# anzeA/Tarok

Measured on AMD Instinct MI355X. Metric: env steps/sec at 65 536 parallel 4-player games; 1/2/4/8 MI355X, higher is better.
Workload: dtype u64

## Files before the change

tarok_amd/csrc/tarok_device.h:

```cpp
#pragma once
#include <hip/hip_runtime.h>
#include <stdint.h>

typedef unsigned long long u64;
typedef uint32_t u32;

#define TK_VGPR_BUDGET(B) __attribute__((amdgpu_num_vgpr((B) - 1)))
#define TK_KERNEL(threads, B) __global__ __launch_bounds__(threads) TK_VGPR_BUDGET(B)
#define TK_VGPR_STR2(x) #x
#define TK_VGPR_STR(x) TK_VGPR_STR2(x)
#define TK_VGPR_TOP(B, TOP)                                                                                           \
    do {                                                                                                              \
        static_assert((B) % 8 == 0 && (B) <= 256 && (TOP) == (B) - 1, "TK_VGPR_TOP(B, B - 1), B a multiple of 8");     \
        asm volatile("" ::: "v" TK_VGPR_STR(TOP));                                                                    \
    } while (0)

#define TK_BIT(i) (1ULL << (i))
#define TK_DECK ((1ULL << 54) - 1)
#define TK_TAROK (((1ULL << 22) - 1) << 32)
#define TK_PAGAT TK_BIT(32)
#define TK_V5 (TK_BIT(7) | TK_BIT(15) | TK_BIT(23) | TK_BIT(31) | TK_BIT(32) | TK_BIT(52) | TK_BIT(53))
#define TK_V4 (TK_BIT(6) | TK_BIT(14) | TK_BIT(22) | TK_BIT(30))
#define TK_V3 (TK_BIT(5) | TK_BIT(13) | TK_BIT(21) | TK_BIT(29))
#define TK_V2 (TK_BIT(4) | TK_BIT(12) | TK_BIT(20) | TK_BIT(28))
// ... 106 lines not shown
        u32 gs = group_size(g.contract);
        return talon_all(g) & ~ids_mask(g.talon, (int)(g.tl * gs), (int)gs);
    }
    return talon_all(g);
}

__device__ __forceinline__ int prestej(u64 m) {
    u32 lo = TK_LO(m), hi = TK_HI(m);
    u32 n = (u32)__popc(lo) + (u32)__popc(hi);
    u32 v = n + (u32)__popc(lo & 0xF0F0F0F0u) + (u32)__popc(lo & 0xE0E0E0E0u) + (u32)__popc(lo & 0xC0C0C0C0u) +
            (u32)__popc(lo & 0x80808080u) + 4u * (u32)__popc(hi & 0x300001u);
    u32 q = (n * 43u) >> 7;
    return (int)(v - 2 * q - (n != 3 * q ? 1u : 0u));
}

__device__ __forceinline__ u32 tk_zero_mask(u32 x) { return (u32)((int)__builtin_amdgcn_sad_u8(x, 0u, ~0u) >> 31); }
__device__ __forceinline__ u64 legal_mask(u64 hand, bool has_lead, u32 lead, u32 contract) {
    u32 hl = TK_LO(hand), hh = TK_HI(hand);
    u32 lm = has_lead ? ~0u : 0u;
    u32 tarok_led = (u32)((int)(lead << 26) >> 31);
    u32 s = TK_BITOP3(hl, 0xFFu << (lead & 24), tarok_led, a_ & b_ & ~c_) & lm;
    u32 zs = tk_zero_mask(s);
    u32 zt = tk_zero_mask(hh) | ~lm;
    u32 bl = s | TK_BITOP3(hl, zs, zt, a_ & b_ & c_);
    u32 bh = hh & zs;
    u32 kf = (0x281u >> contract) & 1u;
    u32 only_pagat = tk_zero_mask(bl | (bh & ~1u));
    return TK_U64(bl, TK_BITOP3(bh, kf, only_pagat, a_ & ~(b_ & ~c_)));
}

__device__ __forceinline__ u64 legal_mask_follow(u64 hand, u32 lead, u32 contract, u32 &hi_sel) {
    u32 hl = TK_LO(hand), hh = TK_HI(hand);
    u32 tarok_led = (u32)((int)(lead << 26) >> 31);
    u32 s = TK_BITOP3(hl, 0xFFu << (lead & 24), tarok_led, a_ & b_ & ~c_);
    u32 zs = tk_zero_mask(s);
    u32 zt = tk_zero_mask(hh);
    u32 bl = s | TK_BITOP3(hl, zs, zt, a_ & b_ & c_);
    u32 bh = hh & zs;
    u32 kf = (0x281u >> contract) & 1u;
    u32 only_pagat = tk_zero_mask(bl | (bh & ~1u));
    hi_sel = TK_BITOP3(zs, zt, zt, a_ & ~b_);           TK_KEEP_VGPR(hi_sel);
    return TK_U64(bl, TK_BITOP3(bh, kf, only_pagat, a_ & ~(b_ & ~c_)));
}

#define TK_FAM_LUT 0xA0000281u
#define TK_FAM_MASK 0x80400001u
struct FamilyWord { u32 w; };
struct LeadWord { u32 m; };
__device__ __forceinline__ FamilyWord family_word(u32 contract) {
    u32 w = (TK_FAM_LUT >> contract) & TK_FAM_MASK;     TK_KEEP_VGPR(w);
    return FamilyWord{w};
}
__device__ __forceinline__ LeadWord lead_word(u32 lead) {
    u32 tarok_led = (u32)((int)(lead << 26) >> 31);     TK_KEEP_VGPR(tarok_led);
    return LeadWord{(0xFFu << (lead & 24)) & ~tarok_led};
}
__device__ __forceinline__ u64 legal_mask(u64 hand, FamilyWord fam) {
    u32 hl = TK_LO(hand), hh = TK_HI(hand);
    u32 only_pagat = tk_zero_mask(hl | (hh & ~1u));
    return TK_U64(hl, TK_BITOP3(hh, fam.w, only_pagat, a_ & ~(b_ & ~c_)));
}
__device__ __forceinline__ u64 legal_mask_follow(u64 hand, LeadWord lead, FamilyWord fam, u32 &hi_sel) {
    u32 hl = TK_LO(hand), hh = TK_HI(hand);
    u32 s = hl & lead.m;
    u32 zs = tk_zero_mask(s);
    u32 zt = tk_zero_mask(hh);
    u32 bl = s | TK_BITOP3(hl, zs, zt, a_ & b_ & c_);
    u32 bh = hh & zs;
    u32 only_pagat = tk_zero_mask(bl | (bh & ~1u));
    hi_sel = TK_BITOP3(zs, zt, zt, a_ & ~b_);           TK_KEEP_VGPR(hi_sel);
    return TK_U64(bl, TK_BITOP3(bh, fam.w, only_pagat, a_ & ~(b_ & ~c_)));
}

__device__ __forceinline__ u64 legal_now(const Game &g) {
    u32 seat = (g.leader + g.nt) & 3;
    return legal_mask(hand_of(g, seat), g.nt != 0, g.trick & 63, g.contract);
}

template <bool IN_PLAY = false>
__device__ __forceinline__ u64 obs_word_with(const Game &g, bool finished_now, u64 legal) {
    u64 o = legal;
    o |= (u64)((g.leader + g.nt) & 3) << 54;
    o |= (u64)(g.trick_no * 4 + g.nt) << 56;
    if (IN_PLAY) o |= (u64)(finished_now ? 1u : 0u) << 62;
    else if (finished_now || g.phase == TK_PHASE_DONE) o |= 1ULL << 62;
    o |= (u64)g.error << 63;
    return o;
}

#define TK_OBS_CARD ((1u << 30) + 1u)
__device__ __forceinline__ u32 obs_carry(u32 seat, u32 pos) { return (seat << 30) | pos; }
__device__ __forceinline__ u32 obs_carry_hi(u32 carry) { return (carry >> 8) | (carry << 24); }
__device__ __forceinline__ u64 obs_word_with(u32 carry, u32 error, u32 fin01, u64 legal) {
    return legal | ((u64)(obs_carry_hi(carry) | (fin01 << 30) | (error << 31)) << 32);
}

__device__ __forceinline__ u32 obs_carry(u32 seat, u32 pos, u32 error) { return (error << 7) | obs_carry(seat, pos); }
__device__ __forceinline__ u32 obs_carry_ma(u32 carry) { return (u32)((int)(carry << 1) >> 31); }
__device__ __forceinline__ u32 obs_carry_mb(u32 carry) { return (u32)((int)carry >> 31); }
__device__ __forceinline__ u64 obs_word_with(u32 carry_with_error, u32 fin01, u64 legal) {
    return legal | ((u64)(obs_carry_hi(carry_with_error) | (fin01 << 30)) << 32);
}

__device__ __forceinline__ u64 obs_word(const Game &g, bool finished_now) {
    bool play = g.phase == TK_PHASE_PLAY;
    u64 o = play ? legal_now(g) : 0;
    o |= (u64)((g.leader + g.nt) & 3) << 54;
    o |= (u64)(g.trick_no * 4 + g.nt) << 56;
    if (finished_now || g.phase == TK_PHASE_DONE) o |= 1ULL << 62;
    o |= (u64)g.error << 63;
    return o;
}

__device__ __forceinline__ u64 pack_scores(int s0, int s1, int s2, int s3) {
    return (u64)(uint16_t)(int16_t)s0 | ((u64)(uint16_t)(int16_t)s1 << 16) |
           ((u64)(uint16_t)(int16_t)s2 << 32) | ((u64)(uint16_t)(int16_t)s3 << 48);
}

__device__ __forceinline__ u64 score_game(const Game &g) {
    bool klop = g.contract == TK_KLOP;
    u64 p0 = pile_of<0>(g), p1 = pile_of<1>(g), p2 = pile_of<2>(g), p3 = pile_of<3>(g);
    u32 t0 = (u32)((int)(g.team << 31) >> 31), t1 = (u32)((int)(g.team << 30) >> 31);
    u32 t2 = (u32)((int)(g.team << 29) >> 31), t3 = (u32)((int)(g.team << 28) >> 31);
    u32 xl = TK_BITOP3(TK_LO(g.A), t1, t0, (a_ & b_) | (~a_ & c_)), yl = TK_BITOP3(TK_LO(g.A), t3, t2, (a_ & b_) | (~a_ & c_));
    u32 xh = TK_BITOP3(TK_HI(g.A), t1, t0, (a_ & b_) | (~a_ & c_)), yh = TK_BITOP3(TK_HI(g.A), t3, t2, (a_ & b_) | (~a_ & c_));
    u32 tl = TK_BITOP3(TK_LO(g.B), yl, xl, (a_ & b_) | (~a_ & c_)) & TK_LO(g.C);
    u32 th = TK_BITOP3(TK_HI(g.B), yh, xh, (a_ & b_) | (~a_ & c_)) & TK_HI(g.C);
    u64 t = TK_U64(tl, th);
    u32 kb = g.king * 8 + 7, d = g.declarer;
    bool king_taken = ((TK_LO(g.C) >> kb) & 1) && ((TK_LO(g.A) >> kb) & 1) == (d & 1) && ((TK_LO(g.B) >> kb) & 1) == (d >> 1);
    bool alone_with_king = !klop && g.contract != TK_SOLO_BREZ && __popc(g.team) == 1 && has_king(g.contract) && king_taken;
    if (alone_with_king) t |= talon_unowned(g);
    int c0 = prestej(klop ? p0 : t), c1 = prestej(klop ? p1 : 0), c2 = prestej(klop ? p2 : 0), c3 = prestej(klop ? p3 : 0);
    bool over = c0 > 35 || c1 > 35 || c2 > 35 || c3 > 35;
    int d0 = c0 - 35, ad = d0 < 0 ? -d0 : d0;
    int r = 5 * (int)(((u32)(ad + 2) * 205u) >> 10);
    if (d0 < 0) r = -r;
    int c = 10 * (int)g.contract;
    int sc = (c0 > 35 ? c : -c) + r;
    int s0 = klop ? (over ? 0 : -c0) : ((g.team & 1) ? sc : 0);
    int s1 = klop ? (over ? 0 : -c1) : ((g.team & 2) ? sc : 0);
    int s2 = klop ? (over ? 0 : -c2) : ((g.team & 4) ? sc : 0);
    int s3 = klop ? (over ? 0 : -c3) : ((g.team & 8) ? sc : 0);
    return pack_scores(s0, s1, s2, s3);
}

__device__ __forceinline__ u64 berac_scores(const Game &g) {
    int v = g.contract == TK_BERAC ? 70 : 90;
    int sc = g.leader == g.declarer ? -v : v;
    u32 d = g.declarer;
    return pack_scores(d == 0 ? sc : 0, d == 1 ? sc : 0, d == 2 ? sc : 0, d == 3 ? sc : 0);
}

template <bool TRUSTED = false, bool DEFER = false, bool CARRIED = false>
__device__ __forceinline__ int apply_step(Game &g, u32 a, u64 &scores, u32 &trick_info, bool want_tv = true, const u64 *c_lead = nullptr,
                                          FamilyWord fam = FamilyWord{0u}, LeadWord lead = LeadWord{0u}) {
    if (!TRUSTED) {
        u64 legal = legal_now(g);
        bool ok = a < 54 && ((legal >> (a & 63)) & 1);
        g.error = ok ? g.error : 1u;
        if (!ok) return -1;
    }
    g.C |= 1ULL << a;
    g.trick |= a << (6 * g.nt);
    g.nt++;
    if (g.nt < 4) return 0;
    u64 tm;
    if (c_lead) tm = g.C ^ *c_lead;
    else {
        u32 c0 = g.trick & 63, c1 = (g.trick >> 6) & 63, c2 = (g.trick >> 12) & 63, c3 = (g.trick >> 18) & 63;
        tm = (1ULL << c0) | (1ULL << c1) | (1ULL << c2) | (1ULL << c3);
    }
    u32 th = TK_HI(tm), tl_ = TK_LO(tm) & (CARRIED ? lead.m : (0xFFu << (g.trick & 24)));
    u32 zt = tk_zero_mask(th);
    u32 wbit = 31u - (u32)__builtin_clz(TK_BITOP3(th, tl_, zt, (a_ & ~c_) | (b_ & c_)));
    u32 aw = TK_BITOP3(TK_HI(g.A), TK_LO(g.A), zt, (a_ & ~c_) | (b_ & c_)), bw = TK_BITOP3(TK_HI(g.B), TK_LO(g.B), zt, (a_ & ~c_) | (b_ & c_));
    u32 ws = __builtin_amdgcn_ubfe(aw, wbit, 1) | (__builtin_amdgcn_ubfe(bw, wbit, 1) << 1);
    {
        u32 gift = CARRIED ? min(g.tl, fam.w >> 31) : (tk_zero_mask(g.contract) & ((g.tl + 7u) >> 3));
        g.tl -= gift;
        u64 gb = 1ULL << ((u32)(g.talon >> (6 * g.tl)) & 63u);
        u32 gm = 0u - gift;
        tm |= TK_U64(TK_LO(gb) & gm, TK_HI(gb) & gm);
    }
    {
        u32 m1 = (u32)((int)(ws << 31) >> 31), m2 = (u32)((int)(ws << 30) >> 31);
        g.A = TK_U64(TK_BITOP3(TK_LO(g.A), TK_LO(tm), m1, (a_ & ~b_) | (b_ & c_)), TK_BITOP3(TK_HI(g.A), TK_HI(tm), m1, (a_ & ~b_) | (b_ & c_)));
        g.B = TK_U64(TK_BITOP3(TK_LO(g.B), TK_LO(tm), m2, (a_ & ~b_) | (b_ & c_)), TK_BITOP3(TK_HI(g.B), TK_HI(tm), m2, (a_ & ~b_) | (b_ & c_)));
    }
    if (want_tv) {
        u32 tv = (u32)(popc64(tm) + popc64(tm & (TK_V2 | TK_V3 | TK_V4 | TK_V5)) + popc64(tm & (TK_V3 | TK_V4 | TK_V5)) +
                       popc64(tm & (TK_V4 | TK_V5)) + popc64(tm & TK_V5)) - 2;
        trick_info = 0x8000u | (tv << 4) | ws;
    }
    g.leader = ws; g.nt = 0; g.trick = 0; g.trick_no++;
    u32 berac01 = CARRIED ? __builtin_amdgcn_ubfe(fam.w, 22u, 1u) : ((0x280u >> g.contract) & 1u);
    u32 over01 = ((g.trick_no + 4u) >> 4) | (berac01 & tk_zero_mask(ws ^ g.declarer));
    if (!DEFER) {
        if (over01) scores = berac01 ? berac_scores(g) : score_game(g);
    }
    g.phase |= over01;
    return (int)over01;
}

__device__ __forceinline__ u64 final_scores(const Game &g) {
    return (g.contract == TK_BERAC || g.contract == TK_ODPRTI_BERAC) ? berac_scores(g) : score_game(g);
}

__device__ __forceinline__ void setup_game(Game &g, u64 h0, u64 h1, u64 h2, u64 h3, u64 talon36,
                                           u32 contract, u32 declarer, u32 king) {
    g.A = h1 | h3; g.B = h2 | h3;
    g.talon = talon36;
    u64 tal = ids_mask(talon36, 0, 6);
    g.C = tal;
    g.trick = 0; g.nt = 0; g.trick_no = 0; g.error = 0;
    g.contract = contract; g.declarer = declarer;
    g.king = has_king(contract) ? king : 0;
    g.leader = (contract == TK_BERAC || contract == TK_ODPRTI_BERAC) ? declarer : 0;
    if (contract == TK_KLOP) {
        g.team = 0; g.tl = 6;
    } else {
        u32 team = 1u << declarer;
        if (has_king(contract)) {
            u64 kb = 1ULL << (king * 8 + 7);
            team |= (h0 & kb) ? 1u : 0u; team |= (h1 & kb) ? 2u : 0u;
            team |= (h2 & kb) ? 4u : 0u; team |= (h3 & kb) ? 8u : 0u;
        }
        g.team = team;
        g.tl = (has_exchange(contract) || contract == TK_SOLO_BREZ) ? 7 : 0;
        u32 o = (u32)__builtin_ctz(~team & 15u);
        g.A |= (o & 1) ? tal : 0;
        g.B |= (o & 2) ? tal : 0;
    }
    g.phase = has_exchange(contract) ? TK_PHASE_EXCHANGE : TK_PHASE_PLAY;
}

__device__ __forceinline__ bool apply_exchange(Game &g, u32 choice, u32 d0, u32 d1, u32 d2) {
    u32 gs = group_size(g.contract);
    u32 ngroups = gs == 3 ? 2u : (gs == 2 ? 3u : 6u);
    u64 grp = ids_mask(g.talon, (int)(choice * gs), (int)gs);
    u64 h = hand_of(g, g.declarer) | grp;
    u32 dpk = (d0 & 255) | ((d1 & 255) << 8) | ((d2 & 255) << 16);
    u64 dm = 0;
    bool ok = choice < ngroups;
#pragma unroll
    for (u32 i = 0; i < 3; i++) {
        u32 di = (dpk >> (8 * i)) & 255;
        bool good = di < 54 && ((h >> (di & 63)) & 1) && !((dm >> (di & 63)) & 1);
        ok = ok && (good || i >= gs);
        dm |= (good && i < gs) ? (1ULL << (di & 63)) : 0;
    }
    u32 s = g.declarer;
    u64 nA = (g.A & ~grp) | ((s & 1) ? grp : 0);
    u64 nB = (g.B & ~grp) | ((s & 2) ? grp : 0);
    u64 nC = (g.C & ~grp) | dm;
    g.A = ok ? nA : g.A;
    g.B = ok ? nB : g.B;
    g.C = ok ? nC : g.C;
    g.tl = ok ? choice : g.tl;
    g.phase = ok ? (u32)TK_PHASE_PLAY : g.phase;
    g.error = ok ? g.error : 1u;
    return ok;
}

__device__ __forceinline__ u64 mix64(u64 x) {
    x ^= x >> 30; x *= 0xBF58476D1CE4E5B9ULL;
    x ^= x >> 27; x *= 0x94D049BB133111EBULL;
    x ^= x >> 31;
    return x;
}
__device__ __forceinline__ u64 game_key(u64 seed, u64 gidx, u64 episode) {
    u64 a = gidx * 0x9E3779B97F4A7C15ULL + episode * 0xD1B54A32D192ED03ULL + 0x2545F4914F6CDD1DULL;
    return mix64(seed ^ mix64(a));
}
#define TK_RNG_STEP 0x9E3779B1u
struct RngCtr { u32 v; };
__device__ __forceinline__ RngCtr rng_ctr(u32 i) { return RngCtr{i * TK_RNG_STEP}; }
__device__ __forceinline__ u32 rng32(u32 lo, u32 hi, RngCtr c) {
    u32 x = lo ^ c.v;
    x ^= x >> 16; x *= 0x85EBCA6Bu;
    x ^= x >> 13; x *= 0xC2B2AE35u;
    x ^= x >> 16; x ^= hi;
    x *= 0x27D4EB2Fu; x ^= x >> 15;
    return x;
}
__device__ __forceinline__ u32 rng32(u32 lo, u32 hi, u32 i) { return rng32(lo, hi, rng_ctr(i)); }
__device__ __forceinline__ u32 rng32(u64 key, u32 i) { return rng32((u32)key, (u32)(key >> 32), i); }
__device__ __forceinline__ u32 rng32(u64 key, RngCtr c) { return rng32((u32)key, (u32)(key >> 32), c); }
__device__ __forceinline__ u32 pick(u32 r, u32 n) { return __umulhi(r, n); }

__device__ __forceinline__ u32 kth_bit(u64 m, u32 k) {
    u32 lo = TK_LO(m), hi = TK_HI(m);
    u32 nk = ~k;
    u32 c = (u32)__popc(lo);
    u32 s0 = (u32)((int)(c + nk) >> 31);
    u32 w = TK_BITOP3(lo, hi, s0, (a_ & ~c_) | (b_ & c_));
    nk += c & s0;
    u32 p = ((u32)__popc(w & 0xFFFFu) + nk) >> 31;
#pragma unroll
    for (int s = 3; s >= 0; s--) {
        u32 q = (p << (s + 1)) | (1u << s);
        u32 d = (u32)__popc(__builtin_amdgcn_ubfe(w, 0, q)) + nk;
        p = (p << 1) | (d >> 31);
    }
    return p | (s0 & 32u);
}

__device__ __forceinline__ u32 kth_bit_word(u32 w, u32 hi_sel, u32 k) {
    u32 nk = ~k;
    u32 p = ((u32)__popc(w & 0xFFFFu) + nk) >> 31;
#pragma unroll
    for (int s = 3; s >= 0; s--) {
        u32 q = (p << (s + 1)) | (1u << s);
        u32 d = (u32)__popc(__builtin_amdgcn_ubfe(w, 0, q)) + nk;
        p = (p << 1) | (d >> 31);
    }
    return p | (hi_sel & 32u);
}

__device__ __forceinline__ u32 policy_action(u64 key, u32 step, u64 mask) {
    return kth_bit(mask, pick(rng32(key, 128 + step), (u32)popc64(mask)));
}
__device__ __forceinline__ u32 policy_action_follow(u64 key, u32 step, u32 w, u32 hi_sel) {
    return kth_bit_word(w, hi_sel, pick(rng32(key, 128 + step), (u32)__popc(w)));
}

__device__ __forceinline__ u32 policy_action(u64 key, RngCtr c, u64 mask) {
    return kth_bit(mask, pick(rng32(key, c), (u32)popc64(mask)));
}
__device__ __forceinline__ u32 policy_action_follow(u64 key, RngCtr c, u32 w, u32 hi_sel) {
    return kth_bit_word(w, hi_sel, pick(rng32(key, c), (u32)__popc(w)));
}

__device__ __forceinline__ void redeal_unseen(Game &g, u32 mover, u64 wkey) {
    const u32 o0 = mover == 0 ? 1u : 0u, o1 = mover <= 1 ? 2u : 1u, o2 = mover == 3 ? 2u : 3u;
    const u64 h0 = hand_of(g, o0), h1 = hand_of(g, o1), h2 = hand_of(g, o2);
    const u64 P = h0 | h1 | h2;
    u32 cap0 = (u32)popc64(h0), cap1 = (u32)popc64(h1), total = (u32)popc64(P);
    u64 m0 = 0, m1 = 0, rest = P;
    const u32 klo = (u32)wkey, khi = (u32)(wkey >> 32), n = total;
    for (u32 i = 0; i < n; i++) {
        u64 bit = rest & (0ULL - rest);
        u32 r = pick(rng32(klo, khi, i), total);
        u32 t0 = r < cap0 ? 1u : 0u, t1 = (r >= cap0 && r < cap0 + cap1) ? 1u : 0u;
        m0 |= t0 ? bit : 0ULL;
        m1 |= t1 ? bit : 0ULL;
        cap0 -= t0; cap1 -= t1; total--;
        rest ^= bit;
    }
    const u64 m2 = P & ~(m0 | m1);
    u64 sa = ((o0 & 1) ? m0 : 0ULL) | ((o1 & 1) ? m1 : 0ULL) | ((o2 & 1) ? m2 : 0ULL);
    u64 sb = ((o0 & 2) ? m0 : 0ULL) | ((o1 & 2) ? m1 : 0ULL) | ((o2 & 2) ? m2 : 0ULL);
    u64 A = (g.A & ~P) | sa, B = (g.B & ~P) | sb;
    const u64 kb = 1ULL << (g.king * 8 + 7);
    const bool hidden = has_king(g.contract) && (P & kb) != 0;
    const u32 got = (m0 & kb) ? o0 : ((m1 & kb) ? o1 : o2);
    const u32 team = hidden ? ((1u << g.declarer) | (1u << got)) : g.team;
    const u64 un = hidden ? talon_unowned(g) : 0ULL;
    const u32 park = (u32)__builtin_ctz((~team & 15u) | 16u);
// ... 589 lines not shown
```

tarok_amd/csrc/tarok_env.hip:

```cpp
#include "tarok_device.h"

#include <hip/hip_runtime.h>
#include <math.h>
#include <stddef.h>
#include <stdint.h>
#include <stdio.h>
#include <stdlib.h>
#include <string.h>
#include <type_traits>
#include <utility>

#include "../../include/tarok_env.h"

#define TK_BLOCK 256
#define TK_PF_SLOTS (4 * TK_BLOCK)
#define TK_GRAPH_CACHE 16
#define TK_REFILL_CAP (TK_BLOCK * TK_AHEAD)
#define TK_REFILL_FAN 8
#define TK_RC(group, k) ((((size_t)(group)) * 4 + (k)) * 32)
#define TK_BULK_EVERY 32u
#define TK_BULK_CAP ((TK_BULK_EVERY / 4) * TK_BLOCK)

#define TK_AHEAD TAROK_GAMES_AHEAD
#define TK_LINE(episode) ((u32)(episode) % (u32)TK_AHEAD)
// ... 222 lines not shown
    u64 o = obs[i], key = gkey[i];
    u64 m = o & TAROK_OBS_MASK;
    u32 a = 255;
    if (m) a = policy_action(key, (u32)(o >> TAROK_OBS_STEP_SHIFT) & 63u, m);
    action[i] = (uint8_t)a;
}

TK_KERNEL(TK_BLOCK, 64) void k_policy_x4(int64_t n, const u64 *__restrict__ obs,
                                                       const u64 *__restrict__ gkey, uint8_t *__restrict__ action) {
    TK_VGPR_TOP(64, 63);
    int64_t base = (int64_t)blockIdx.x * (4 * TK_BLOCK);
    if (base + 4 * TK_BLOCK <= n) {
        int64_t p0 = base + 2 * threadIdx.x, p1 = p0 + 2 * TK_BLOCK;
        ulonglong2 o0 = *reinterpret_cast<const ulonglong2 *>(obs + p0), o1 = *reinterpret_cast<const ulonglong2 *>(obs + p1);
        ulonglong2 k0 = *reinterpret_cast<const ulonglong2 *>(gkey + p0), k1 = *reinterpret_cast<const ulonglong2 *>(gkey + p1);
        auto one = [](u64 o, u64 key) __attribute__((always_inline)) {
            u64 m = o & TAROK_OBS_MASK;
            return m ? policy_action(key, (u32)(o >> TAROK_OBS_STEP_SHIFT) & 63u, m) : 255u;
        };
        u32 a0 = one(o0.x, k0.x) | (one(o0.y, k0.y) << 8), a1 = one(o1.x, k1.x) | (one(o1.y, k1.y) << 8);
        *reinterpret_cast<uint16_t *>(action + p0) = (uint16_t)a0;
        *reinterpret_cast<uint16_t *>(action + p1) = (uint16_t)a1;
        return;
    }
    for (int64_t i = base + threadIdx.x; i < n; i += TK_BLOCK) {
        u64 o = obs[i];
        u64 m = o & TAROK_OBS_MASK;
        u32 a = 255;
        if (m) a = policy_action(gkey[i], (u32)(o >> TAROK_OBS_STEP_SHIFT) & 63u, m);
        action[i] = (uint8_t)a;
    }
}

template <class T> __device__ __forceinline__ T tk_ld(const T *p) { return __hip_atomic_load(p, __ATOMIC_RELAXED, __HIP_MEMORY_SCOPE_AGENT); }

#define TK_EPOCH_SHARDS 256
#define TK_EPOCH_WORDS (32 * TK_EPOCH_SHARDS)
#define TK_PHASES (2u * TK_BULK_EVERY)
static_assert((TK_BULK_EVERY & (TK_BULK_EVERY - 1)) == 0 && TK_BULK_EVERY >= 4 && TK_BULK_EVERY + 1 <= 4 * (TK_AHEAD - 1),
              "a line is dealt at most TK_BULK_EVERY + 1 launches after it was emptied and is needed again TK_AHEAD - 1 games (four launches each, at least) after that");
struct TkCount { u32 own, other; };
__device__ __forceinline__ u32 tk_shard_size(u32 grid, u32 shard) { return (grid + TK_EPOCH_SHARDS - 1 - shard) / TK_EPOCH_SHARDS; }
template <int KIND> __device__ __forceinline__ u32 tk_other_grid(u32 groups, u32 fan) { return KIND == 0 ? groups + (groups + fan - 1) / fan : groups; }
template <int KIND> __device__ __forceinline__ u32 tk_other_shard(u32 groups) { return (KIND == 0 ? blockIdx.x : blockIdx.x % groups) % TK_EPOCH_SHARDS; }
template <int KIND> __device__ __forceinline__ TkCount launch_count(const u32 *epoch, u32 groups) {
    TkCount c;
    c.own = tk_ld(epoch + KIND * TK_EPOCH_WORDS + 32 * (blockIdx.x % TK_EPOCH_SHARDS));
    c.other = tk_ld(epoch + (1 - KIND) * TK_EPOCH_WORDS + 32 * tk_other_shard<KIND>(groups));
    return c;
}
__device__ __forceinline__ u32 tk_div_small(u32 count, u32 g) {
    u32 q = (u32)(((float)count + 0.5f) * __builtin_amdgcn_rcpf((float)g));
    q -= (q * g > count) ? 1u : 0u;
    q += ((q + 1u) * g <= count) ? 1u : 0u;
    return q;
}
template <int KIND> __device__ __forceinline__ u32 launch_phase(TkCount c, u32 groups, u32 fan) {
    asm volatile("" : "+v"(c.own), "+v"(c.other));
    u32 own = tk_div_small(c.own, tk_shard_size(gridDim.x, blockIdx.x % TK_EPOCH_SHARDS));
    u32 other = tk_div_small(c.other, tk_shard_size(tk_other_grid<KIND>(groups, fan), tk_other_shard<KIND>(groups)));
    return (own + other) % TK_PHASES;
}
template <int KIND> __device__ __forceinline__ void launch_counted(u32 *epoch) {
    if (threadIdx.x == 0)
        (void)atomicInc(epoch + KIND * TK_EPOCH_WORDS + 32 * (blockIdx.x % TK_EPOCH_SHARDS),
                        TK_PHASES * tk_shard_size(gridDim.x, blockIdx.x % TK_EPOCH_SHARDS) - 1u);
}

template <bool BULK>
__device__ __forceinline__ void refill_role(u32 rblock, u32 tid, u32 nthreads, u64 seed, u64 offset, int mix, u32 play_groups,
                                        TkCount count, u32 *epoch, u32 fan, bool bulk_on, Aux *aux, u64 *rlist, u32 *rcount, u64 *elist) {
    constexpr int KIND = BULK ? 0 : 1;
    const u32 kind_fan = fan;
    if (BULK) fan = 1;
    u32 g0 = rblock * fan;
    u32 len0[TK_REFILL_FAN], len1[TK_REFILL_FAN];
#pragma unroll
    for (u32 q = 0; q < TK_REFILL_FAN; q++) {
        bool has = q < fan && g0 + q < play_groups;
        len0[q] = has ? tk_ld(&rcount[TK_RC(g0 + q, 0)]) : 0u;
        len1[q] = has ? tk_ld(&rcount[TK_RC(g0 + q, 1)]) : 0u;
    }
    if (!BULK) {
        __syncthreads();
        launch_counted<KIND>(epoch);
    }
    const u32 phase = launch_phase<KIND>(count, play_groups, kind_fan), par = phase & 1u;
    if (!BULK) {
        if (tid < 2 * fan && g0 + tid / 2 < play_groups) rcount[TK_RC(g0 + tid / 2, 2 + (tid & 1))] = 0u;
    }
    u32 cum[TK_REFILL_FAN + 1];
    cum[0] = 0;
    u32 which = par ^ 1u;
    const u32 odd = 0u - par;
#pragma unroll
    for (u32 q = 0; q < TK_REFILL_FAN; q++) cum[q + 1] = cum[q] + ((len0[q] & odd) | (len1[q] & ~odd));
    const bool any = cum[TK_REFILL_FAN] != 0;
    u64 *lists = rlist;
    u32 cap = TK_REFILL_CAP;
    const bool bulk = BULK && bulk_on && phase % TK_BULK_EVERY == 0;
#pragma nounroll
    for (u32 pass = 0; pass < (BULK ? 2u : 1u); pass++) {
        if (pass == 1) {
            if (!bulk) break;
            which = ((phase / TK_BULK_EVERY) & 1u) ^ 1u;
            lists = elist; cap = TK_BULK_CAP;
#pragma unroll
            for (u32 q = 0; q < TK_REFILL_FAN; q++) {
                bool has = q < fan && g0 + q < play_groups;
                cum[q + 1] = cum[q] + (has ? min(tk_ld(&rcount[TK_RC(g0 + q, 2 + which)]), (u32)TK_BULK_CAP) : 0u);
            }
        }
        for (u32 j = tid; j < cum[TK_REFILL_FAN]; j += nthreads) {
            u32 q = 0;
#pragma unroll
            for (u32 r = 1; r < TK_REFILL_FAN; r++) q += j >= cum[r] ? 1u : 0u;
            u32 base = 0;
#pragma unroll
            for (u32 r = 0; r < TK_REFILL_FAN; r++) base = (r == q) ? cum[r] : base;
            u64 en = tk_ld(&lists[((int64_t)(g0 + q) * 2 + which) * cap + (j - base)]);
            deal_into_buffer(aux, (int64_t)(g0 + q) * TK_BLOCK + (u32)(en & 0xFFFF), (u32)(en >> 32), seed, offset, mix);
        }
    }
    if (any || bulk) {
        __syncthreads();
        if (any && tid < fan && g0 + tid < play_groups) rcount[TK_RC(g0 + tid, par ^ 1u)] = 0u;
        if (bulk && tid < fan && g0 + tid < play_groups) rcount[TK_RC(g0 + tid, 2 + which)] = 0u;
    }
}

template <bool HIST>
__device__ __forceinline__ void play_role(
    u32 group, u32 tid,
    int64_t n, u64 seed, u64 offset, int mix, int flags, int cards, int64_t stride, TkCount count, u32 *epoch, u32 play_groups, u32 fan,
    uint8_t *__restrict__ action_out, int16_t *__restrict__ reward,
    uint8_t *__restrict__ done, uint16_t *__restrict__ trick, u64 *__restrict__ obs, uint8_t *__restrict__ hist,
    ulonglong2 *__restrict__ s01, ulonglong2 *__restrict__ s23, Aux *aux, Counters *__restrict__ cnt,
    u64 *__restrict__ gkey, u64 *rlist, u32 *rcount, u64 *__restrict__ stamps) {
    __shared__ unsigned short push_list[TK_REFILL_CAP];
    __shared__ u32 push_ep[TK_BLOCK];
    __shared__ u32 push_count;
    __shared__ u32 finq[TK_BLOCK / 64][9][TK_FINQ];
    __shared__ int sacc[4][TK_BLOCK];
    if (tid == 0) push_count = 0;
    sacc[0][tid] = 0; sacc[1][tid] = 0; sacc[2][tid] = 0; sacc[3][tid] = 0;
    __syncthreads();
    u32 fq_head = 0, fq_n = 0;
    u32 (*fq)[TK_FINQ] = finq[tid >> 6];
    auto drain_finished = [&](u32 cnt_) __attribute__((always_inline)) {
        u32 lane = tid & 63;
        if (lane < cnt_) {
            u32 e = (fq_head + lane) & (TK_FINQ - 1);
            Game f;
            f.A = TK_U64(fq[0][e], fq[1][e]); f.B = TK_U64(fq[2][e], fq[3][e]); f.C = TK_U64(fq[4][e], fq[5][e] & 0x3FFFFFu);
            u32 m = fq[7][e], ri = fq[8][e];
            f.talon = TK_U64(fq[6][e], (m >> 24) & 15u);
            f.contract = m & 15; f.declarer = (m >> 4) & 3; f.king = (m >> 6) & 3; f.team = (m >> 8) & 15;
            f.tl = (m >> 12) & 7; f.trick_no = (m >> 16) & 15; f.leader = (m >> 20) & 3;
            f.trick = 0; f.nt = 0; f.phase = TK_PHASE_DONE; f.error = 0; f.epar = 0; f.cprev = 0;
            u64 sc = final_scores(f);
            u32 t = ri & 0xFFFFu;
            if (reward) {
                u64 rs = sc;
                if ((flags & TAROK_REWARD_REF) && (f.contract == TK_BERAC || f.contract == TK_ODPRTI_BERAC)) {
                    int dv = f.trick_no >= 12 ? -20 : 20;
                    u32 d = f.declarer;
                    rs = pack_scores(d == 0 ? (int)(int16_t)(sc & 0xFFFF) : dv, d == 1 ? (int)(int16_t)((sc >> 16) & 0xFFFF) : dv,
                                     d == 2 ? (int)(int16_t)((sc >> 32) & 0xFFFF) : dv, d == 3 ? (int)(int16_t)(sc >> 48) : dv);
                }
                reinterpret_cast<u64 *>(reward)[(int64_t)group * TK_BLOCK + t + (int64_t)(ri >> 16) * stride] = rs;
            }
            atomicAdd(&sacc[0][t], (int)(int16_t)(sc & 0xFFFF)); atomicAdd(&sacc[1][t], (int)(int16_t)((sc >> 16) & 0xFFFF));
            atomicAdd(&sacc[2][t], (int)(int16_t)((sc >> 32) & 0xFFFF)); atomicAdd(&sacc[3][t], (int)(int16_t)(sc >> 48));
        }
        fq_head = (fq_head + cnt_) & (TK_FINQ - 1);
        fq_n -= cnt_;
    };
    u64 t_real0 = 0, t_cyc0 = 0, t_play = 0;
    if (stamps) { t_real0 = __builtin_amdgcn_s_memrealtime(); t_cyc0 = __builtin_amdgcn_s_memtime(); }
    int64_t i = (int64_t)group * TK_BLOCK + tid;
    bool valid = i < n;
    int64_t ic = valid ? i : n - 1;
    Game g;
    load_game(g, s01, s23, ic);
    u64 key = gkey[ic];
    bool autoreset = (flags & TAROK_AUTO_RESET) != 0;
    bool berac = g.contract == TK_BERAC || g.contract == TK_ODPRTI_BERAC;
    bool spec = valid && ((g.phase == TK_PHASE_PLAY && (int)g.nt + cards >= 4 &&
                           (berac || (int)(g.trick_no * 4 + g.nt) + cards >= 48)) ||
                          g.phase == TK_PHASE_DONE);
    u32 cprev0 = valid ? g.cprev : 0u;
    u32 allowed = TK_AHEAD - min(cprev0, (u32)TK_AHEAD);
    int4 acc = make_int4(0, 0, 0, 0);
    u32 cur_ep = 0;
    ulonglong2 na = make_ulonglong2(0, 0), nb = na, na2 = na, nb2 = na;
    u64 nkey = 0, nkey2 = 0;
    u32 nep1 = 0, nep2 = 0;
    bool ok1 = false, ok2 = false;
    auto line_tag = [&](bool &ok, u32 &nep, u32 tag) __attribute__((always_inline)) { nep = tag; ok = true; };
    static_assert(offsetof(AuxLine, nkey) == 32 && offsetof(AuxLine, nep) == 40, "key and tag share the line's third 16 bytes");
    auto load_line = [&](const AuxLine *ln, ulonglong2 &a, ulonglong2 &b, u64 &k, bool &ok, u32 &nep) __attribute__((always_inline)) {
        a = ln->n01; b = ln->n23;
        uint3 kt = *reinterpret_cast<const uint3 *>(__builtin_assume_aligned(&ln->nkey, 16));
        k = TK_U64(kt.x, kt.y);
        line_tag(ok, nep, kt.z);
    };
    const bool all_play = autoreset && __ballot(valid && g.phase == TK_PHASE_PLAY) == ~0ULL;
    const bool aligned = all_play && (cards & 3) == 0 && __ballot(g.nt != 0) == 0 &&
                         (u64)stride <= 0xFFFFFFFFull && (u64)stride * (u32)cards + (u64)n <= 0xFFFFFFFFull;
    if (spec) {
        acc = cnt[i].score_sum;
        cur_ep = cnt[i].episode;
        if (autoreset && allowed > 0) {
            load_line(&aux[i].line[TK_LINE(g.epar + 1)], na, nb, nkey, ok1, nep1);
            if (!aligned && allowed > 1 && cards > 4)
                load_line(&aux[i].line[TK_LINE(g.epar + 2)], na2, nb2, nkey2, ok2, nep2);
        }
    }
    TK_WAIT_LOADS();
    u32 par = launch_phase<1>(count, play_groups, fan) & 1u;
    launch_counted<1>(epoch);
    g.cprev = 0;
    u32 consumed = 0;
    bool resync = false;
    bool blocked = false;
    bool acc_dirty = false, seats_dirty = false, touched = false;
    u64 legal = (valid && g.phase == TK_PHASE_PLAY) ? legal_now(g) : 0;
    u64 c_lead = 0;
    u32 legal_hi = 0;
    u32 rctr = 0, ocar = 0;
    FamilyWord fam = FamilyWord{0u};
    LeadWord led = LeadWord{0u};
    u32 resync_v = 0;
    u32 lim = spec ? allowed : 0u;
    u32 out_b = (u32)i;
    u64 *out_obs = obs + i;
    auto fetch_lines = [&](bool lacks, bool lacks2) __attribute__((always_inline)) {
        if (lacks) load_line(&aux[i].line[TK_LINE(cur_ep + 1)], na, nb, nkey, ok1, nep1);
        if (lacks2) load_line(&aux[i].line[TK_LINE(cur_ep + 2)], na2, nb2, nkey2, ok2, nep2);
    };
    auto play_card = [&](auto all_tag, auto nt_tag, auto std_tag, int64_t row, int ci) __attribute__((always_inline)) {
        constexpr bool ALL = decltype(all_tag)::value;
        constexpr int NT = decltype(nt_tag)::value;
        constexpr bool STD = decltype(std_tag)::value;
        if constexpr (NT >= 0) g.nt = (u32)NT;
        constexpr bool TOP_UP_EARLY = ALL && NT == 0;
        constexpr bool TOP_UP_LATE = !(ALL && NT == 3);
        if constexpr (TOP_UP_EARLY) {
            if (nep1 != cur_ep + 1 && consumed < lim) {
                u32 off = g.epar + 1 >= (u32)TK_AHEAD ? 0u : (g.epar + 1) * (u32)sizeof(AuxLine);
                load_line(reinterpret_cast<const AuxLine *>(reinterpret_cast<const char *>(aux[i].line) + off), na, nb, nkey, ok1, nep1);
            }
        }
        const bool v = ALL ? true : valid;
        const bool play = ALL ? true : (valid && g.phase == TK_PHASE_PLAY);
        constexpr bool ALIGNED = ALL && NT >= 0;
        u32 a;
        if constexpr (ALL && NT >= 1) a = policy_action_follow(key, RngCtr{rctr}, TK_LO(legal) | TK_HI(legal), legal_hi);
        else if constexpr (ALIGNED) a = policy_action(key, RngCtr{rctr}, legal);
        else a = play ? policy_action(key, g.trick_no * 4 + g.nt, legal) : 255u;
        if constexpr (ALIGNED) rctr += TK_RNG_STEP;
        u64 scores = 0;
        u32 trick_info = 0;
        int res = -2;
        const u32 pos = g.trick_no * 4 + g.nt;
        if constexpr (ALL && NT == 0) c_lead = g.C;
        const u64 *lead_plane = (ALL && NT >= 0) ? &c_lead : nullptr;
        if constexpr (ALL && NT == 0) led = lead_word(a);
        if constexpr (ALIGNED) res = apply_step<true, true, true>(g, a, scores, trick_info, !STD && trick != nullptr, lead_plane, fam, led);
        else if (play) res = apply_step<true, true>(g, a, scores, trick_info, !STD && trick != nullptr, lead_plane);
        bool fin = res == 1;
        if (HIST && hist && play && res >= 0) hist[(int64_t)pos * n + i] = (uint8_t)a;
        if constexpr (!(ALL && NT >= 0)) {
            touched = touched || res != -2;
            seats_dirty = seats_dirty || (res >= 0 && g.nt == 0);
        }
        if constexpr (ALIGNED) {
            if (STD || action_out) TK_STREAM_STORE(&action_out[out_b], (uint8_t)a);
            if (!STD && trick) TK_STREAM_STORE(&trick[out_b], (uint16_t)trick_info);
        } else if (v) {
            if (STD || action_out) TK_STREAM_STORE(&action_out[row], (uint8_t)a);
            if (!STD && trick) TK_STREAM_STORE(&trick[row], (uint16_t)trick_info);
        }
        constexpr bool CAN_END = !(ALL && NT >= 0 && NT < 3);
        constexpr bool FAST_RENEW = ALL && NT == 3;
        auto push_finished = [&](u64 fm, u32 slot0) __attribute__((always_inline)) {
            u32 e = (slot0 + __builtin_amdgcn_mbcnt_hi((u32)(fm >> 32), __builtin_amdgcn_mbcnt_lo((u32)fm, 0))) & (TK_FINQ - 1);
            fq[0][e] = TK_LO(g.A); fq[1][e] = TK_HI(g.A); fq[2][e] = TK_LO(g.B); fq[3][e] = TK_HI(g.B);
            fq[4][e] = TK_LO(g.C); fq[5][e] = TK_HI(g.C); fq[6][e] = TK_LO(g.talon);
            u32 m = (g.declarer << 4) | g.contract;      TK_KEEP_VGPR(m);
            m = (g.king << 6) | m;                       TK_KEEP_VGPR(m);
            m = (g.team << 8) | m;                       TK_KEEP_VGPR(m);
            m = (g.tl << 12) | m;                        TK_KEEP_VGPR(m);
            m = (g.trick_no << 16) | m;                  TK_KEEP_VGPR(m);
            m = (g.leader << 20) | m;                    TK_KEEP_VGPR(m);
            fq[7][e] = (TK_HI(g.talon) << 24) | m;
            fq[8][e] = ((u32)ci << 16) | tid;
        };
        auto swap_in = [&]() __attribute__((always_inline)) {
            unpack_fresh(g, na.x, na.y, nb.x, nb.y);
            if constexpr (ALIGNED) g.C |= TK_C_PAD;
            key = nkey;
            if constexpr (!ALIGNED) {
                na = na2; nb = nb2; nkey = nkey2;
                nep1 = nep2;
            }
        };
        auto deal_in_place = [&](bool deal_here, Game &gd, u64 &kd) __attribute__((always_inline)) {
            u64 pend = __ballot(deal_here);
            if (TK_RARE(pend != 0)) {
                u64 dkey = 0;
                if (deal_here) dkey = game_key(seed, offset + (u64)i, cur_ep + 1);
                u64 h0 = 0, h1 = 0, h2 = 0, h3 = 0, tal = 0;
                u32 lane = __lane_id();
                while (pend) {
                    int l = __builtin_ctzll(pend);
                    pend &= pend - 1;
                    u32 klo = (u32)__builtin_amdgcn_readlane((int)(u32)dkey, l);
                    u32 khi = (u32)__builtin_amdgcn_readlane((int)(u32)(dkey >> 32), l);
                    u64 w0, w1, w2, w3, wt;
                    deal_wave(klo, khi, w0, w1, w2, w3, wt);
                    if (lane == (u32)l) { h0 = w0; h1 = w1; h2 = w2; h3 = w3; tal = wt; }
                }
                if (deal_here) {
                    u32 cc, d, k;
                    sample_setup(dkey, mix, cc, d, k);
                    setup_game(gd, h0, h1, h2, h3, tal, cc, d, k);
                    gd.epar = TK_LINE(cur_ep + 1); gd.cprev = 0;
                    if (gd.phase == TK_PHASE_EXCHANGE) bot_exchange(gd, dkey);
                    kd = dkey;
                }
            }
        };
        if constexpr (FAST_RENEW) {
            u64 fm = __ballot(fin);
            const u64 nol = __ballot(nep1 != cur_ep + 1);
            if (TK_USUAL(fm != 0)) {
                if (TK_RARE(fq_n >= 64)) drain_finished(64);
                const u32 slot0 = fq_head + fq_n;
                fq_n += (u32)__popcll(fm);
                if (TK_RARE((fm & nol) != 0)) {
                    bool lineless = fin && nep1 != cur_ep + 1;
                    resync_v |= (lineless && consumed < lim) ? 1u : 0u;
                    lim = lineless ? 0u : lim;
                    Game d = g;
                    u64 dk = key;
                    deal_in_place(lineless, d, dk);
                    if (lineless) { pack(d, na.x, na.y, nb.x, nb.y); nkey = dk; nep1 = cur_ep + 1; }
                }
                if (fin) { push_finished(fm, slot0); swap_in(); cur_ep++; consumed++; rctr = rng_ctr(128u).v; fam = family_word(g.contract); }
            }
        }
        if constexpr (CAN_END && !FAST_RENEW) {
            u64 fm = __ballot(fin);
            if (TK_USUAL(fm != 0)) {
                if (TK_RARE(fq_n >= 64)) drain_finished(64);
                if (fin) push_finished(fm, fq_head + fq_n);
                fq_n += (u32)__popcll(fm);
            }
        }
        if (CAN_END && !FAST_RENEW && (ALL || autoreset)) {
            bool renew = ALL ? fin : (v && g.phase == TK_PHASE_DONE);
            if (TK_USUAL(__ballot(renew) != 0)) {
                if constexpr (TOP_UP_LATE) {
                    bool lacks = spec && !blocked && !ok1 && consumed >= 1 && consumed < allowed;
                    if (TK_RARE(__ballot(renew && lacks) != 0)) {
                        bool lacks2 = spec && !blocked && !ok2 && consumed >= 1 && consumed + 1 < allowed;
                        fetch_lines(lacks, lacks2);
                        TK_WAIT_LOADS();
                    }
                }
                bool swap = renew && !blocked && ok1 && nep1 == cur_ep + 1;
                if (swap) {
                    swap_in();
                    ok1 = ok2 && consumed + 1 < allowed;
                    ok2 = false;
                }
                bool deal_here = renew && !swap;
                if (deal_here && consumed < allowed) resync = true;
                if (deal_here) blocked = true;
                deal_in_place(deal_here, g, key);
                if (renew) { cur_ep++; consumed++; seats_dirty = true; }
            }
        }
        if constexpr (ALIGNED && NT < 3) ocar += TK_OBS_CARD;
        else if constexpr (ALIGNED) ocar = obs_carry(g.leader, g.trick_no << 2, g.error);
        if constexpr (ALIGNED && NT < 3) legal = legal_mask_follow(hand_of<true>(g, obs_carry_ma(ocar), obs_carry_mb(ocar)), led, fam, legal_hi);
        else if constexpr (ALIGNED) legal = legal_mask(hand_of<true>(g, obs_carry_ma(ocar), obs_carry_mb(ocar)), fam);
        else legal = (ALL || (v && g.phase == TK_PHASE_PLAY)) ? legal_now(g) : 0;
        const u32 fin01 = ALL ? (u32)res : (fin ? 1u : 0u);
        if constexpr (ALIGNED) {
            TK_STREAM_STORE(out_obs, obs_word_with(ocar, fin01, legal));
            if (STD || done) TK_STREAM_STORE(&done[out_b], (uint8_t)fin01);
            out_b += (u32)stride; out_obs += stride;
        } else if (v) {
            TK_STREAM_STORE(&obs[row], obs_word_with<true>(g, false, legal) | ((u64)(ALL ? fin01 : ((fin || g.phase == TK_PHASE_DONE) ? 1u : 0u)) << 62));
            if (STD || done) TK_STREAM_STORE(&done[row], (uint8_t)fin01);
        }
    };
    int64_t row = i;
    typedef std::integral_constant<int, -1> nt_any;
    if (all_play) {
        if (aligned) {
            auto tricks = [&](auto std_tag) __attribute__((always_inline)) {
                touched = true; seats_dirty = true;
                g.C |= TK_C_PAD;
                rctr = rng_ctr(128u + g.trick_no * 4).v;
                ocar = obs_carry(g.leader, g.trick_no << 2, g.error);
                fam = family_word(g.contract);
                for (int c = 0; c < cards; c += 4) {
                    play_card(std::true_type{}, std::integral_constant<int, 0>{}, std_tag, row, c);
                    play_card(std::true_type{}, std::integral_constant<int, 1>{}, std_tag, row, c + 1);
                    play_card(std::true_type{}, std::integral_constant<int, 2>{}, std_tag, row, c + 2);
                    play_card(std::true_type{}, std::integral_constant<int, 3>{}, std_tag, row, c + 3);
                }
                g.C &= TK_DECK;
            };
            if (action_out && done && !trick) tricks(std::true_type{});
            else tricks(std::false_type{});
        } else {
            for (int c = 0; c < cards; c++, row += stride) play_card(std::true_type{}, nt_any{}, std::false_type{}, row, c);
        }
    } else {
        for (int c = 0; c < cards; c++, row += stride) play_card(std::false_type{}, nt_any{}, std::false_type{}, row, c);
    }
    while (fq_n) drain_finished(min(fq_n, 64u));
    __builtin_amdgcn_s_waitcnt(0xC07F);
    {
        int4 sa = make_int4(sacc[0][tid], sacc[1][tid], sacc[2][tid], sacc[3][tid]);
        if (sa.x | sa.y | sa.z | sa.w) { acc.x += sa.x; acc.y += sa.y; acc.z += sa.z; acc.w += sa.w; acc_dirty = true; }
    }
    u32 np = (resync || resync_v != 0) ? (u32)TK_AHEAD : min(consumed, (u32)TK_AHEAD);
    if (valid) {
        g.cprev = np;
        if (acc_dirty) cnt[i].score_sum = acc;
        if (consumed) { cnt[i].episode = cur_ep; gkey[i] = key; }
        if (touched || consumed || cprev0 != np) store_game(g, s01, s23, i, seats_dirty || cprev0 != np);
    }
    if (stamps) t_play = __builtin_amdgcn_s_memtime() - t_cyc0;
    if (valid && np) {
        u32 pos = atomicAdd(&push_count, np);
        push_ep[tid] = cur_ep;
        for (u32 j = 0; j < np; j++) push_list[pos + j] = (unsigned short)(j * TK_BLOCK + tid);
    }
    __syncthreads();
    u32 total = push_count;
    u64 *lst = rlist + ((int64_t)group * 2 + par) * TK_REFILL_CAP;
    for (u32 j = tid; j < total; j += TK_BLOCK) {
        u32 en = push_list[j], t = en % TK_BLOCK;
        lst[j] = ((u64)(push_ep[t] + TK_AHEAD - en / TK_BLOCK) << 32) | t;
    }
    if (tid == 0) rcount[TK_RC(group, par)] = total;
    if (stamps && (tid & 63) == 0) {
        u64 w = (u64)i >> 6;
        stamps[3 * w + 0] = t_real0;
        stamps[3 * w + 1] = __builtin_amdgcn_s_memrealtime();
        stamps[3 * w + 2] = ((__builtin_amdgcn_s_memtime() - t_cyc0) << 32) | (t_play & 0xFFFFFFFFULL);
    }
}

#define TK_PLAY_ARGS                                                                                                             \
    int64_t n, u64 seed, u64 offset, int mix, int flags, int cards, int64_t stride, u32 play_groups, u32 *epoch, u32 fan,         \
        uint8_t *__restrict__ action_out, int16_t *__restrict__ reward,                                                           \
        uint8_t *__restrict__ done, uint16_t *__restrict__ trick, u64 *__restrict__ obs, uint8_t *__restrict__ hist,              \
        ulonglong2 *__restrict__ s01, ulonglong2 *__restrict__ s23, Aux *aux, Counters *__restrict__ cnt,                         \
        u64 *__restrict__ gkey, u64 *rlist, u32 *rcount, u64 *__restrict__ stamps
template <bool HIST>
TK_KERNEL(TK_BLOCK, 168) __attribute__((amdgpu_waves_per_eu(3, 3))) void k_play_wide(TK_PLAY_ARGS) {
    TK_VGPR_TOP(168, 167);
    TkCount count = launch_count<1>(epoch, play_groups);
    if (blockIdx.x >= play_groups)
        refill_role<false>(blockIdx.x - play_groups, threadIdx.x, TK_BLOCK, seed, offset, mix, play_groups, count, epoch, fan, false, aux, rlist, rcount, nullptr);
    else {
        play_role<HIST>(blockIdx.x, threadIdx.x, n, seed, offset, mix, flags, cards, stride, count, epoch, play_groups, fan,
                        action_out, reward, done, trick, obs, hist, s01, s23, aux, cnt, gkey, rlist, rcount, stamps);
    }
}

__device__ __forceinline__ void deal_in_place_wave(bool deal_here, Game &gd, u64 &kd, u64 seed, u64 offset, int64_t i, u32 ep, int mix) {
    u64 pend = __ballot(deal_here);
    if (pend == 0) return;
    u64 dkey = 0;
    if (deal_here) dkey = game_key(seed, offset + (u64)i, ep);
    u64 h0 = 0, h1 = 0, h2 = 0, h3 = 0, tal = 0;
    u32 lane = __lane_id();
    while (pend) {
        int l = __builtin_ctzll(pend);
        pend &= pend - 1;
        u32 klo = (u32)__builtin_amdgcn_readlane((int)(u32)dkey, l);
        u32 khi = (u32)__builtin_amdgcn_readlane((int)(u32)(dkey >> 32), l);
        u64 w0, w1, w2, w3, wt;
        deal_wave(klo, khi, w0, w1, w2, w3, wt);
        if (lane == (u32)l) { h0 = w0; h1 = w1; h2 = w2; h3 = w3; tal = wt; }
    }
    if (deal_here) {
        u32 cc, d, k;
        sample_setup(dkey, mix, cc, d, k);
        setup_game(gd, h0, h1, h2, h3, tal, cc, d, k);
        gd.epar = TK_LINE(ep); gd.cprev = 0;
        if (gd.phase == TK_PHASE_EXCHANGE) bot_exchange(gd, dkey);
        kd = dkey;
    }
}

#define FINQ_WORDS 13
template <bool RANDOM, bool LAZY>
__device__ __forceinline__ void step_role(
    u32 group, u32 tid, bool active, u32 a_reg, bool lazy_on,
    int64_t n, u64 seed, u64 offset, int mix, int flags, TkCount count, u32 *epoch, u32 play_groups, u32 fan,
    const uint8_t *__restrict__ action_in, uint8_t *__restrict__ action_out, int16_t *__restrict__ reward,
    uint8_t *__restrict__ done, uint16_t *__restrict__ trick, u64 *__restrict__ obs, uint8_t *__restrict__ hist,
    ulonglong2 *__restrict__ s01, ulonglong2 *__restrict__ s23, Aux *aux, Counters *__restrict__ cnt,
    u64 *__restrict__ gkey, u64 *rlist, u32 *rcount, u64 *elist,
    u32 (*__restrict__ finq)[TK_BLOCK] ) {
    __shared__ unsigned short push_list[TK_REFILL_CAP];
    __shared__ u32 push_ep[TK_BLOCK];
    __shared__ u32 push_count, fin_count, late_count;
    __shared__ u64 late_list[LAZY ? TK_BLOCK : 1];
    const bool lazy = LAZY && lazy_on;
    if (tid == 0) { push_count = 0; fin_count = 0; late_count = 0; }
    u32 efill0 = 0, efill1 = 0;
    if (lazy) { efill0 = tk_ld(&rcount[TK_RC(group, 2)]); efill1 = tk_ld(&rcount[TK_RC(group, 3)]); }
    __syncthreads();
    int64_t i = (int64_t)group * TK_BLOCK + tid;
    bool valid = active && i < n;
    int64_t ic = valid ? i : n - 1;
    Game g;
    load_game(g, s01, s23, ic);
    u64 key = 0;
    u32 a = 255;
    if (RANDOM) key = gkey[ic]; else a = action_in ? action_in[ic] : a_reg;
    const bool autoreset = (flags & TAROK_AUTO_RESET) != 0;
    const u32 cprev0 = valid ? g.cprev : 0u;
    const u32 allowed = TK_AHEAD - min(cprev0, (u32)TK_AHEAD);
    int4 acc = make_int4(0, 0, 0, 0);
    u32 cur_ep = 0;
    ulonglong2 na = make_ulonglong2(0, 0), nb = na;
    u64 nkey = 0;
    u32 ntag = 0;
    bool have_line = false;
    auto load_finish = [&](bool need) __attribute__((always_inline)) {
        if (need) {
            acc = cnt[i].score_sum;
            cur_ep = cnt[i].episode;
            if (autoreset && allowed > 0) {
                const AuxLine *ln = &aux[i].line[TK_LINE(g.epar + 1)];
                na = ln->n01; nb = ln->n23; nkey = ln->nkey; ntag = ln->nep;
                have_line = true;
            }
        }
    };
    launch_counted<LAZY ? 0 : 1>(epoch);
    g.cprev = 0;
    const bool play = valid && g.phase == TK_PHASE_PLAY;
    const u32 pos = g.trick_no * 4 + g.nt;
    if (RANDOM) a = play ? policy_action(key, pos, legal_now(g)) : 255u;
    u64 scores = 0;
    u32 trick_info = 0;
    int res = -2;
    if (play) res = apply_step<RANDOM, true>(g, a, scores, trick_info, trick != nullptr, nullptr);
    const bool fin = res == 1;
    if (hist && play && res >= 0) hist[(int64_t)pos * n + i] = (uint8_t)a;
    bool seats_dirty = res >= 0 && g.nt == 0;
    if (valid) {
        if (RANDOM && action_out) TK_STREAM_STORE(&action_out[i], (uint8_t)a);
        if (trick) TK_STREAM_STORE(&trick[i], (uint16_t)trick_info);
    }
    const bool renew = autoreset && valid && g.phase == TK_PHASE_DONE;
    load_finish(fin || renew);
// ... 3034 lines not shown
```

Before: 201.5 billion.

## Pack per-game seat metadata into spare high bits of card planes

During the aligned all-play trick loop, contract, declarer, king, team and epar are folded into the unused bits above bit 54 of the A and B card planes and unpacked only at loop exit. Readers in the hot loop (berac over-check, family word, epar line offset, finished-queue write) pull fields with bitfield extracts. Fresh game swap-in uses a seats-aware unpack. The aim is to cut live VGPRs under the tight VGPR budget. The cost is extra masking, and any code that reads A/B without masking the high bits risks wrong results.

```diff
diff --git a/tarok_amd/csrc/tarok_device.h b/tarok_amd/csrc/tarok_device.h
--- a/tarok_amd/csrc/tarok_device.h
+++ b/tarok_amd/csrc/tarok_device.h
@@ -282,7 +282,7 @@
     return pack_scores(d == 0 ? sc : 0, d == 1 ? sc : 0, d == 2 ? sc : 0, d == 3 ? sc : 0);
 }
 
-template <bool TRUSTED = false, bool DEFER = false, bool CARRIED = false>
+template <bool TRUSTED = false, bool DEFER = false, bool CARRIED = false, bool SEATS = false>
 __device__ __forceinline__ int apply_step(Game &g, u32 a, u64 &scores, u32 &trick_info, bool want_tv = true, const u64 *c_lead = nullptr,
                                           FamilyWord fam = FamilyWord{0u}, LeadWord lead = LeadWord{0u}) {
     if (!TRUSTED) {
@@ -325,7 +325,8 @@
     }
     g.leader = ws; g.nt = 0; g.trick = 0; g.trick_no++;
     u32 berac01 = CARRIED ? __builtin_amdgcn_ubfe(fam.w, 22u, 1u) : ((0x280u >> g.contract) & 1u);
-    u32 over01 = ((g.trick_no + 4u) >> 4) | (berac01 & tk_zero_mask(ws ^ g.declarer));
+    u32 declarer = SEATS ? __builtin_amdgcn_ubfe(TK_HI(g.A), 26u, 2u) : g.declarer;
+    u32 over01 = ((g.trick_no + 4u) >> 4) | (berac01 & tk_zero_mask(ws ^ declarer));
     if (!DEFER) {
         if (over01) scores = berac01 ? berac_scores(g) : score_game(g);
     }
@@ -335,6 +336,51 @@
 
 __device__ __forceinline__ u64 final_scores(const Game &g) {
     return (g.contract == TK_BERAC || g.contract == TK_ODPRTI_BERAC) ? berac_scores(g) : score_game(g);
+}
+
+#define TK_SEATS_A(contract, declarer, king) ((contract) | ((declarer) << 4) | ((king) << 6))
+#define TK_SEATS_B(team, epar) ((team) | ((epar) << 4))
+__device__ __forceinline__ u32 seats_contract(const Game &g) { return __builtin_amdgcn_ubfe(TK_HI(g.A), 22u, 4u); }
+__device__ __forceinline__ u32 seats_declarer(const Game &g) { return __builtin_amdgcn_ubfe(TK_HI(g.A), 26u, 2u); }
+__device__ __forceinline__ u32 seats_epar(const Game &g) { return __builtin_amdgcn_ubfe(TK_HI(g.B), 26u, 4u); }
+__device__ __forceinline__ void seats_into_planes(Game &g) {
+    g.A |= (u64)TK_SEATS_A(g.contract, g.declarer, g.king) << 54;
+    g.B |= (u64)TK_SEATS_B(g.team, g.epar) << 54;
+}
+__device__ __forceinline__ void seats_out_of_planes(Game &g) {
+    u32 m2 = TK_HI(g.A) >> 22, m3 = TK_HI(g.B) >> 22;
+    g.contract = m2 & 15; g.declarer = (m2 >> 4) & 3; g.king = (m2 >> 6) & 3;
+    g.team = m3 & 15; g.epar = (m3 >> 4) & 15;
+    g.A &= TK_DECK; g.B &= TK_DECK;
+}
+__device__ __forceinline__ void unpack_fresh_seats(Game &g, u64 x0, u64 x1, u64 y0, u64 y1) {
+    g.C = x0 | TK_C_PAD; g.A = y0; g.B = y1;
+    u32 m0 = (u32)(x0 >> 54);
+    g.nt = 0; g.leader = (m0 >> 2) & 3; g.trick_no = 0; g.phase = m0 >> 8;
+    g.talon = x1 & ((1ULL << 36) - 1);
+    g.trick = 0;
+    g.tl = (u32)(x1 >> 60) & 7; g.error = (u32)(x1 >> 63);
+    g.cprev = 0;
+}
+
+template <bool SEATS>
+__device__ __forceinline__ void fin_entry_write(const Game &g, u32 (&w)[8]) {
+    w[0] = TK_LO(g.A); w[2] = TK_LO(g.B);
+    w[1] = SEATS ? TK_HI(g.A) : (TK_HI(g.A) | (TK_SEATS_A(g.contract, g.declarer, g.king) << 22));
+    w[3] = SEATS ? TK_HI(g.B) : (TK_HI(g.B) | (TK_SEATS_B(g.team, 0u) << 22));
+    w[4] = TK_LO(g.C); w[5] = TK_HI(g.C); w[6] = TK_LO(g.talon);
+    u32 m = g.tl << 12;                          TK_KEEP_VGPR(m);
+    m = (g.trick_no << 16) | m;                  TK_KEEP_VGPR(m);
+    m = (g.leader << 20) | m;                    TK_KEEP_VGPR(m);
+    w[7] = (TK_HI(g.talon) << 24) | m;
+}
+__device__ __forceinline__ void fin_entry_read(Game &f, const u32 (&w)[8]) {
+    u32 m2 = w[1] >> 22, m3 = w[3] >> 22, m = w[7];
+    f.A = TK_U64(w[0], w[1] & 0x3FFFFFu); f.B = TK_U64(w[2], w[3] & 0x3FFFFFu); f.C = TK_U64(w[4], w[5] & 0x3FFFFFu);
+    f.talon = TK_U64(w[6], (m >> 24) & 15u);
+    f.contract = m2 & 15; f.declarer = (m2 >> 4) & 3; f.king = (m2 >> 6) & 3; f.team = m3 & 15;
+    f.tl = (m >> 12) & 7; f.trick_no = (m >> 16) & 15; f.leader = (m >> 20) & 3;
+    f.trick = 0; f.nt = 0; f.phase = TK_PHASE_DONE; f.error = 0; f.epar = 0; f.cprev = 0;
 }
 
 __device__ __forceinline__ void setup_game(Game &g, u64 h0, u64 h1, u64 h2, u64 h3, u64 talon36,
diff --git a/tarok_amd/csrc/tarok_env.hip b/tarok_amd/csrc/tarok_env.hip
--- a/tarok_amd/csrc/tarok_env.hip
+++ b/tarok_amd/csrc/tarok_env.hip
@@ -398,12 +398,9 @@
         if (lane < cnt_) {
             u32 e = (fq_head + lane) & (TK_FINQ - 1);
             Game f;
-            f.A = TK_U64(fq[0][e], fq[1][e]); f.B = TK_U64(fq[2][e], fq[3][e]); f.C = TK_U64(fq[4][e], fq[5][e] & 0x3FFFFFu);
-            u32 m = fq[7][e], ri = fq[8][e];
-            f.talon = TK_U64(fq[6][e], (m >> 24) & 15u);
-            f.contract = m & 15; f.declarer = (m >> 4) & 3; f.king = (m >> 6) & 3; f.team = (m >> 8) & 15;
-            f.tl = (m >> 12) & 7; f.trick_no = (m >> 16) & 15; f.leader = (m >> 20) & 3;
-            f.trick = 0; f.nt = 0; f.phase = TK_PHASE_DONE; f.error = 0; f.epar = 0; f.cprev = 0;
+            const u32 w[8] = {fq[0][e], fq[1][e], fq[2][e], fq[3][e], fq[4][e], fq[5][e], fq[6][e], fq[7][e]};
+            const u32 ri = fq[8][e];
+            fin_entry_read(f, w);
             u64 sc = final_scores(f);
             u32 t = ri & 0xFFFFu;
             if (reward) {
@@ -494,7 +491,8 @@
         constexpr bool TOP_UP_LATE = !(ALL && NT == 3);
         if constexpr (TOP_UP_EARLY) {
             if (nep1 != cur_ep + 1 && consumed < lim) {
-                u32 off = g.epar + 1 >= (u32)TK_AHEAD ? 0u : (g.epar + 1) * (u32)sizeof(AuxLine);
+                const u32 ep1 = seats_epar(g) + 1;
+                u32 off = ep1 >= (u32)TK_AHEAD ? 0u : ep1 * (u32)sizeof(AuxLine);
                 load_line(reinterpret_cast<const AuxLine *>(reinterpret_cast<const char *>(aux[i].line) + off), na, nb, nkey, ok1, nep1);
             }
         }
@@ -513,7 +511,7 @@
         if constexpr (ALL && NT == 0) c_lead = g.C;
         const u64 *lead_plane = (ALL && NT >= 0) ? &c_lead : nullptr;
         if constexpr (ALL && NT == 0) led = lead_word(a);
-        if constexpr (ALIGNED) res = apply_step<true, true, true>(g, a, scores, trick_info, !STD && trick != nullptr, lead_plane, fam, led);
+        if constexpr (ALIGNED) res = apply_step<true, true, true, true>(g, a, scores, trick_info, !STD && trick != nullptr, lead_plane, fam, led);
         else if (play) res = apply_step<true, true>(g, a, scores, trick_info, !STD && trick != nullptr, lead_plane);
         bool fin = res == 1;
         if (HIST && hist && play && res >= 0) hist[(int64_t)pos * n + i] = (uint8_t)a;
@@ -532,20 +530,15 @@
         constexpr bool FAST_RENEW = ALL && NT == 3;
         auto push_finished = [&](u64 fm, u32 slot0) __attribute__((always_inline)) {
             u32 e = (slot0 + __builtin_amdgcn_mbcnt_hi((u32)(fm >> 32), __builtin_amdgcn_mbcnt_lo((u32)fm, 0))) & (TK_FINQ - 1);
-            fq[0][e] = TK_LO(g.A); fq[1][e] = TK_HI(g.A); fq[2][e] = TK_LO(g.B); fq[3][e] = TK_HI(g.B);
-            fq[4][e] = TK_LO(g.C); fq[5][e] = TK_HI(g.C); fq[6][e] = TK_LO(g.talon);
-            u32 m = (g.declarer << 4) | g.contract;      TK_KEEP_VGPR(m);
-            m = (g.king << 6) | m;                       TK_KEEP_VGPR(m);
-            m = (g.team << 8) | m;                       TK_KEEP_VGPR(m);
-            m = (g.tl << 12) | m;                        TK_KEEP_VGPR(m);
-            m = (g.trick_no << 16) | m;                  TK_KEEP_VGPR(m);
-            m = (g.leader << 20) | m;                    TK_KEEP_VGPR(m);
-            fq[7][e] = (TK_HI(g.talon) << 24) | m;
+            u32 w[8];
+            fin_entry_write<ALIGNED>(g, w);
+            fq[0][e] = w[0]; fq[1][e] = w[1]; fq[2][e] = w[2]; fq[3][e] = w[3];
+            fq[4][e] = w[4]; fq[5][e] = w[5]; fq[6][e] = w[6]; fq[7][e] = w[7];
             fq[8][e] = ((u32)ci << 16) | tid;
         };
         auto swap_in = [&]() __attribute__((always_inline)) {
-            unpack_fresh(g, na.x, na.y, nb.x, nb.y);
-            if constexpr (ALIGNED) g.C |= TK_C_PAD;
+            if constexpr (ALIGNED) unpack_fresh_seats(g, na.x, na.y, nb.x, nb.y);
+            else unpack_fresh(g, na.x, na.y, nb.x, nb.y);
             key = nkey;
             if constexpr (!ALIGNED) {
                 na = na2; nb = nb2; nkey = nkey2;
@@ -590,11 +583,13 @@
                     resync_v |= (lineless && consumed < lim) ? 1u : 0u;
                     lim = lineless ? 0u : lim;
                     Game d = g;
+                    d.contract = 0; d.declarer = 0; d.king = 0; d.team = 0; d.epar = 0;
+                    d.A &= TK_DECK; d.B &= TK_DECK; d.C &= TK_DECK;
                     u64 dk = key;
                     deal_in_place(lineless, d, dk);
                     if (lineless) { pack(d, na.x, na.y, nb.x, nb.y); nkey = dk; nep1 = cur_ep + 1; }
                 }
-                if (fin) { push_finished(fm, slot0); swap_in(); cur_ep++; consumed++; rctr = rng_ctr(128u).v; fam = family_word(g.contract); }
+                if (fin) { push_finished(fm, slot0); swap_in(); cur_ep++; consumed++; rctr = rng_ctr(128u).v; fam = family_word(seats_contract(g)); }
             }
         }
         if constexpr (CAN_END && !FAST_RENEW) {
@@ -651,6 +646,7 @@
             auto tricks = [&](auto std_tag) __attribute__((always_inline)) {
                 touched = true; seats_dirty = true;
                 g.C |= TK_C_PAD;
+                seats_into_planes(g);
                 rctr = rng_ctr(128u + g.trick_no * 4).v;
                 ocar = obs_carry(g.leader, g.trick_no << 2, g.error);
                 fam = family_word(g.contract);
@@ -661,6 +657,7 @@
                     play_card(std::true_type{}, std::integral_constant<int, 3>{}, std_tag, row, c + 3);
                 }
                 g.C &= TK_DECK;
+                seats_out_of_planes(g);
             };
             if (action_out && done && !trick) tricks(std::true_type{});
             else tricks(std::false_type{});
```

After: 202.2 billion, median of 6. Within noise of the previous version (+0.4%).
